# coop-columb/two-tower-amazon-recommender

Hardware: AMD Instinct MI355X
Metric: user-item pairs/sec (train step) + embedding-gather HBM GB/s, 1/2/4/8 MI355X (higher is better)
Workload: dtype f32; 1 GPU; cfg3: 5000000 users x 10000000 items, emb_dim 128, towers 128->256->128, batch 8192, in-batch sampled softmax T=0.1, sgd lr 1e-3, ids U; global_batch=8192, parallelism=single GPU

## Files before the change

two_tower_amazon_recommender_amd/csrc/score.hip:

```cpp
#include "common.h"

namespace {

using tt::f32x4;
using tt::f32x16;
typedef __bf16 bf16x4 __attribute__((ext_vector_type(4)));
typedef __bf16 bf16x8 __attribute__((ext_vector_type(8)));
typedef short s16x4 __attribute__((ext_vector_type(4)));

constexpr float kLog2e = 1.44269504088896340736f;
constexpr float kLn2 = 0.69314718055994530942f;
constexpr float kNegBig = -1.0e30f;

enum { MODE_FWD = 0, MODE_BWD = 1, MODE_FUSED = 2, MODE_RANK = 3, MODE_FUSED_S = 4, MODE_BWD_S = 5,
       MODE_FUSED_S_NC = 6, MODE_BWD_S_NR = 7 };
constexpr int base_mode(int m) { return m == MODE_FUSED_S_NC ? (int)MODE_FUSED_S : (m == MODE_BWD_S_NR ? (int)MODE_BWD_S : m); }
template <bool B> struct BoolC { static constexpr bool value = B; };
constexpr float kRescaleThr = 8.0f;

struct ScoreArgs {
  const float* R;
  const float* K;
  int64_t n_r, n_c;
  int64_t diag;
  float c1;
  const float* a_r;
  const float* s_r;
  const float* a_c;
  const float* s_c;
  const int64_t* id_r;
  const int64_t* id_c;
  int nsplit;
  int64_t c_per_split;
  float* part_m;
  float* part_l;
  float* pos2;
  float* slab;
  const float* h_r;
  const float* h_c;
  const int64_t* pos_idx;
  int32_t* part_cnt;
  float* S;
  int64_t ldS;
};

template <int D, int PREC>
struct Geo {
  static constexpr int LS = D + 4;
  static constexpr int NG = D / 8;
  static constexpr int NB = D / 32;
  static constexpr int KS = D / 16;
  static constexpr int HALF_B = 32 * 256;
  static constexpr int PIECE_B = (D / 128) * HALF_B;
  static constexpr int TILE_F = PREC == 0 ? 32 * LS : 3 * PIECE_B / 4;
  static constexpr int BUF_F = TILE_F + 160;
  static constexpr int LDS_BYTES = 2 * BUF_F * 4;
};

struct Bf3 {
  __bf16 hi, mid, lo;
};
__device__ __forceinline__ Bf3 split3(float x) {
  Bf3 o;
  o.hi = (__bf16)x;
  const float r1 = x - (float)o.hi;
  o.mid = (__bf16)r1;
  o.lo = (__bf16)(r1 - (float)o.mid);
  return o;
}

__device__ __forceinline__ int img_off(int row, int ch) { return 256 * row + 16 * (ch ^ (((row & 3) << 2) | ((row >> 2) & 3))); }

constexpr int kBwdSWaves = 2;
constexpr int kSPrefetch = 2;
#ifndef TT_LOOP_LAMBDA
#define TT_LOOP_LAMBDA 0
#endif
constexpr int kTilesPerBarrier = 2;
constexpr int kTilesPerBarrierBwdS = kTilesPerBarrier;
template <int D, int MODE, int PREC>
constexpr int tiles_per_barrier() {
  if (PREC == 0 && D <= 128 && MODE == MODE_BWD_S) return kTilesPerBarrierBwdS;
  return (PREC == 0 && D <= 128 && (MODE == MODE_BWD || MODE == MODE_FUSED || MODE == MODE_FUSED_S))
             ? kTilesPerBarrier : 1;
}

template <int D, int MODE, int PREC>
constexpr bool split_d() {
  return PREC == 1 && D == 256 && (MODE == MODE_BWD || MODE == MODE_FUSED || MODE == MODE_FUSED_S);
}
template <int D, int MODE, bool HAS_IDS, bool HAS_HN, int PREC>
constexpr int rf_lds_groups() {
  if (PREC == 0 && D == 256 && (MODE == MODE_FUSED || MODE == MODE_FUSED_S) && (HAS_IDS || HAS_HN))
    return (HAS_IDS && HAS_HN) ? 10 : (HAS_HN ? 8 : 5);
  if (PREC == 0 && D == 128 && MODE == MODE_BWD && HAS_IDS && HAS_HN) return 2;
  return 0;
}
template <int D, int MODE, int PREC, int WAVES>
constexpr int rows_per_wg() { return (split_d<D, MODE, PREC>() ? WAVES / 2 : WAVES) * 32; }

template <int D, int MODE_T, bool HAS_IDS, bool HAS_HN, int WAVES, int PREC>
__global__ __launch_bounds__(WAVES * 64, (WAVES == 8 ? 2 : (D <= 128 ? ((base_mode(MODE_T) == MODE_BWD_S && PREC == 0) ? kBwdSWaves : 2) : 1))) void score_kernel(ScoreArgs p) {
  constexpr int MODE = base_mode(MODE_T);
  constexpr bool FAST = MODE_T != MODE;
  static_assert(!FAST || (PREC == 0 && !HAS_IDS && !HAS_HN), "the fast forms: exact f32, no ids, no hard negatives");
  constexpr BoolC<false> GEN{};
  constexpr BoolC<true> FULL_TILE{};
  constexpr bool NO_AC = FAST && MODE == MODE_FUSED_S;
  constexpr bool NO_ROW = FAST && MODE == MODE_BWD_S;
  constexpr bool IS_FUSED = MODE == MODE_FUSED || MODE == MODE_FUSED_S;
  constexpr bool IS_BWD = MODE == MODE_BWD || MODE == MODE_BWD_S;
  constexpr bool FROM_S = MODE == MODE_BWD_S, TO_S = MODE == MODE_FUSED_S;
  using G_ = Geo<D, PREC>;
  constexpr int LS = G_::LS, NG = G_::NG, NB = G_::NB, TILE_F = G_::TILE_F, BUF_F = G_::BUF_F;
  constexpr int HALF_B = G_::HALF_B, PIECE_B = G_::PIECE_B;
  constexpr bool SPLIT = split_d<D, MODE, PREC>();
  constexpr int KS = SPLIT ? G_::KS / 2 : G_::KS;
  constexpr int NBW = SPLIT ? NB / 2 : NB;
  static_assert(PREC == 0 || D % 128 == 0, "bf16x3: dim 128 / 256 only (whole [32][128] bf16 images)");
  constexpr int ROW4 = D / 4;
  constexpr int THREADS = WAVES * 64;
  constexpr int NV = (32 * ROW4 + THREADS - 1) / THREADS;
  extern __shared__ __attribute__((aligned(16))) float smem[];

  const int tid = threadIdx.x;
  const int lane = tid & 63;
  const int wave = FAST ? __builtin_amdgcn_readfirstlane(tid >> 6) : tid >> 6;
  const int h = lane >> 5;
  const int ln = lane & 31;

  const int split = __builtin_amdgcn_readfirstlane((int)(blockIdx.x % (unsigned)p.nsplit));
  const int64_t rblk = __builtin_amdgcn_readfirstlane((int)(blockIdx.x / (unsigned)p.nsplit));
  const int hw = SPLIT ? (wave & 1) : 0;
  const int64_t r0w = rblk * rows_per_wg<D, MODE, PREC, WAVES>() + (SPLIT ? wave >> 1 : wave) * 32;
  const int64_t r = r0w + ln;
  const bool r_ok = r < p.n_r;
  const int64_t c_begin = (int64_t)split * p.c_per_split;
  int64_t c_end = c_begin + p.c_per_split;
  if (c_end > p.n_c) c_end = p.n_c;
  const int ntiles = __builtin_amdgcn_readfirstlane(c_end > c_begin ? (int)((c_end - c_begin + 31) >> 5) : 0);
  const int nfull = __builtin_amdgcn_readfirstlane(c_end > c_begin ? (int)((c_end - c_begin) >> 5) : 0);

// ... 40 lines not shown
  }
  const float ar = (!NO_ROW && (IS_BWD || MODE == MODE_RANK) && p.a_r != nullptr && r_ok) ? p.a_r[r] : 0.f;
  const float sr = (!NO_ROW && IS_BWD && p.s_r != nullptr && r_ok) ? p.s_r[r] : 1.f;
  int64_t idr = 0;
  if constexpr (HAS_IDS) idr = r_ok ? p.id_r[r] : (int64_t)-1;
  const int64_t cpos = p.pos_idx != nullptr ? (r_ok ? p.pos_idx[r] : (int64_t)-1) : r + p.diag;

  f32x4 st[NV];
  float st_a = 0.f, st_s = 0.f, st_h = -3.0e38f;
  constexpr bool hn = HAS_HN;
  const float hr = (HAS_HN && p.h_r != nullptr && r_ok) ? p.h_r[r] : -3.0e38f;
  int64_t st_id = -2;
  constexpr int RPJ = THREADS / ROW4 > 0 ? THREADS / ROW4 : 1;
  const int st_row = tid / ROW4, st_col4 = tid % ROW4;
  const f32x4* kp = reinterpret_cast<const f32x4*>(p.K) + c_begin * ROW4;
  const bool has_ac = p.a_c != nullptr, has_sc = p.s_c != nullptr, has_hc = HAS_HN && p.h_c != nullptr;
  const float* acp = (has_ac ? p.a_c : p.K) + c_begin;
  const float* scp = (has_sc ? p.s_c : p.K) + c_begin;
  const float* hcp = (has_hc ? p.h_c : p.K) + c_begin;
  const int64_t* idp = nullptr;
  if constexpr (HAS_IDS) idp = p.id_c + c_begin;
  const int ncols = (int)(c_end - c_begin);

  constexpr bool ST_FULL = NV * THREADS == 32 * ROW4;
  auto load_tile = [&](int t, auto full) {
    constexpr bool FULL = decltype(full)::value;
    const f32x4* src = kp + (int64_t)t * (32 * ROW4);
    if constexpr (FULL) {
      static_assert(ST_FULL || NV == 1, "threads past row 31 exist only where a thread stages one float4");
      const unsigned off0 = (unsigned)((ST_FULL ? st_row : (st_row < 31 ? st_row : 31)) * ROW4 + st_col4);
#pragma unroll
      for (int j = 0; j < NV; ++j) st[j] = (src + (ST_FULL ? j * RPJ * ROW4 : 0))[off0];
      const unsigned c31 = (unsigned)(tid < 31 ? tid : 31);
      if constexpr (!NO_AC) st_a = (acp + 32 * (int64_t)t)[c31];
      if constexpr (IS_BWD) st_s = (scp + 32 * (int64_t)t)[c31];
      return;
    }
    const int nvalid = ncols - 32 * t;
    const int last = (nvalid < 32 ? nvalid : 32) - 1;
#pragma unroll
    for (int j = 0; j < NV; ++j) {
      const int row = st_row + j * RPJ;
      st[j] = src[(row < last ? row : last) * ROW4 + st_col4];
    }
    const int c = 32 * t + (tid < last ? tid : last);
    if constexpr (!NO_AC) st_a = acp[c];
    if constexpr (HAS_HN) st_h = hcp[c];
    if constexpr (IS_BWD) st_s = scp[c];
    if constexpr (HAS_IDS) st_id = idp[c];
  };
  auto store_tile = [&](int t, int buf, auto full) {
    constexpr bool FULL = decltype(full)::value;
    float* T = smem + buf * BUF_F;
    const int nvalid = ncols - 32 * t;
    if constexpr (!FULL) {
#pragma unroll
      for (int j = 0; j < NV; ++j) st[j] = (st_row + j * RPJ < nvalid) ? st[j] : f32x4{0.f, 0.f, 0.f, 0.f};
    }
    if constexpr (!ST_FULL) {
#pragma unroll
      for (int j = 0; j < NV; ++j) asm volatile("" : : "v"(st[j]));
    }
    if constexpr (PREC == 0) {
      float* dst = T + st_row * LS + st_col4 * 4;
#pragma unroll
      for (int j = 0; j < NV; ++j)
        if (ST_FULL || st_row + j * RPJ < 32) *reinterpret_cast<f32x4*>(dst + j * RPJ * LS) = st[j];
    } else {
      char* img = reinterpret_cast<char*>(T);
      const int d0 = 4 * st_col4;
      const int sub = (d0 >> 7) * HALF_B + 8 * ((d0 >> 2) & 1), ch = (d0 & 127) >> 3;
#pragma unroll
      for (int j = 0; j < NV; ++j) {
        const int row = st_row + j * RPJ;
        if (ST_FULL || row < 32) {
          bf16x4 q0, q1, q2;
#pragma unroll
          for (int e = 0; e < 4; ++e) {
            const Bf3 u = split3(st[j][e]);
            q0[e] = u.hi; q1[e] = u.mid; q2[e] = u.lo;
          }
          char* dst = img + sub + img_off(row, ch);
          *reinterpret_cast<bf16x4*>(dst) = q0;
          *reinterpret_cast<bf16x4*>(dst + PIECE_B) = q1;
          *reinterpret_cast<bf16x4*>(dst + 2 * PIECE_B) = q2;
        }
      }
    }
    if constexpr (NO_AC) {
      return;
    } else if constexpr (NO_ROW) {
      asm volatile("" : : "v"(st_a));
      asm volatile("" : : "v"(st_s));
      if (tid < 32) {
        const bool ok = FULL || tid < nvalid;
        T[TILE_F + tid] = ok ? st_a : kNegBig;
        T[TILE_F + 32 + tid] = ok ? st_s : 0.f;
      }
      return;
    }
    asm volatile("" : : "v"(st_a));
    if constexpr (IS_BWD) asm volatile("" : : "v"(st_s));
    if constexpr (HAS_HN) asm volatile("" : : "v"(st_h));
    if constexpr (HAS_IDS) asm volatile("" : : "v"(st_id));
    if (tid < 32) {
      const bool ok = tid < nvalid;
      T[TILE_F + tid] = ok ? (has_ac ? st_a : 0.f) : kNegBig;
      T[TILE_F + 32 + tid] = ok ? ((IS_BWD && has_sc) ? st_s : 1.f) : 0.f;
      if constexpr (HAS_HN) T[TILE_F + 128 + tid] = (ok && has_hc) ? st_h : -3.0e38f;
      if constexpr (HAS_IDS) reinterpret_cast<int64_t*>(T + TILE_F + 64)[tid] = ok ? st_id : (int64_t)-2;
    }
  };

  const bool frag_ok = __builtin_amdgcn_readfirstlane((int)(r0w < p.n_r)) != 0;
  auto store_S = [&](int t, const f32x16& X) {
    if (!frag_ok) return;
    const int64_t ctile = (c_begin >> 5) + t;
    if constexpr (FAST) {
      float* blk_u = p.S + (ctile * p.ldS + (r0w >> 5)) * 1024;
      const unsigned lo = (unsigned)(ln * 32 + 4 * h);
#pragma unroll
      for (int g = 0; g < 4; ++g) *reinterpret_cast<f32x4*>(blk_u + (lo + 8u * g)) = f32x4{X[4 * g], X[4 * g + 1], X[4 * g + 2], X[4 * g + 3]};
// ... 10 lines not shown
    f32x4* mine = reinterpret_cast<f32x4*>(xch + wave * 1024) + lane;
    const f32x4* other = reinterpret_cast<const f32x4*>(xch + (wave ^ 1) * 1024) + lane;
#pragma unroll
    for (int g = 0; g < 4; ++g) mine[64 * g] = f32x4{X[4 * g], X[4 * g + 1], X[4 * g + 2], X[4 * g + 3]};
    __syncthreads();
#pragma unroll
    for (int g = 0; g < 4; ++g) {
      const f32x4 o = other[64 * g];
#pragma unroll
      for (int i = 0; i < 4; ++i) X[4 * g + i] += o[i];
    }
  };
  auto load_S = [&](int t, f32x16& X) {
    const int64_t q0 = c_begin + 32 * (int64_t)t;
    if constexpr (FAST) {
      const float* blk_u = p.S + ((frag_ok ? (r0w >> 5) : 0) * p.ldS + (q0 >> 5)) * 1024;
      const unsigned lo = (unsigned)(4 * h * 32 + ln);
#pragma unroll
      for (int reg = 0; reg < 16; ++reg) X[reg] = blk_u[lo + (unsigned)(tt::acc_row(reg, 0) * 32)];
      return;
    }
    const float* blk = p.S + ((frag_ok ? (r0w >> 5) : 0) * p.ldS + (q0 >> 5)) * 1024 + 4 * h * 32 + ln;
#pragma unroll
    for (int reg = 0; reg < 16; ++reg) X[reg] = blk[tt::acc_row(reg, 0) * 32];
  };
  auto mask_S = [&](int t, const f32x16& Xin) -> f32x16 {
    const int nq_left = ncols - 32 * t;
    f32x16 X;
#pragma unroll
    for (int reg = 0; reg < 16; ++reg) X[reg] = (r_ok && (tt::acc_row(reg, 0) + 4 * h) < nq_left) ? Xin[reg] : 0.f;
    return X;
  };
  auto clamp_tile = [&](int t) { return t < ntiles ? t : ntiles - 1; };

  float run_m = kNegBig, run_l = 0.f, pos = 0.f;
  int cnt = 0;
  bool have_pos = false;
  f32x16 G[NBW];
  if constexpr (IS_BWD || IS_FUSED) {
#pragma unroll
    for (int b = 0; b < NBW; ++b)
#pragma unroll
      for (int i = 0; i < 16; ++i) G[b][i] = 0.f;
  }

#pragma unroll
  for (int t0 = 0; t0 < TPB; ++t0)
    if (t0 < ntiles) {
      load_tile(t0, GEN);
      store_tile(t0, t0, GEN);
    }
  __syncthreads();
  auto gemm1 = [&](const float* T) -> f32x16 {
    f32x16 X;
#pragma unroll
    for (int i = 0; i < 16; ++i) X[i] = 0.f;
    if constexpr (PREC == 1) {
      const char* img = reinterpret_cast<const char*>(T);
      auto frag = [&](int ks, bf16x8& f_hi, bf16x8& f_mid, bf16x8& f_lo, bf16x8& r_lo) {
        const int off = (SPLIT ? hw : (ks >> 3)) * HALF_B + img_off(ln, 2 * (ks & 7) + h);
        f_hi = *reinterpret_cast<const bf16x8*>(img + off);
        f_mid = *reinterpret_cast<const bf16x8*>(img + PIECE_B + off);
        f_lo = *reinterpret_cast<const bf16x8*>(img + 2 * PIECE_B + off);
        if constexpr (RLO_LDS) r_lo = rlo[ks * 64];
      };
      bf16x8 a_hi, a_mid, a_lo, b_lo = {};
// ... 6 lines not shown
        X = __builtin_amdgcn_mfma_f32_32x32x16_bf16(a_lo, rp[0][ks], X, 0, 0, 0);
        X = __builtin_amdgcn_mfma_f32_32x32x16_bf16(a_hi, b_lo, X, 0, 0, 0);
        X = __builtin_amdgcn_mfma_f32_32x32x16_bf16(a_mid, rp[1][ks], X, 0, 0, 0);
        X = __builtin_amdgcn_mfma_f32_32x32x16_bf16(a_mid, rp[0][ks], X, 0, 0, 0);
        X = __builtin_amdgcn_mfma_f32_32x32x16_bf16(a_hi, rp[1][ks], X, 0, 0, 0);
        X = __builtin_amdgcn_mfma_f32_32x32x16_bf16(a_hi, rp[0][ks], X, 0, 0, 0);
        a_hi = n_hi; a_mid = n_mid; a_lo = n_lo; b_lo = nb_lo;
        __builtin_amdgcn_sched_barrier(0);
      }
    } else {
      const float* arow = T + ln * LS + 4 * h;
      f32x4 a_cur = *reinterpret_cast<const f32x4*>(arow);
#pragma unroll
      for (int g = 0; g < NG; ++g) {
        f32x4 a_nxt = a_cur;
        if (g + 1 < NG) a_nxt = *reinterpret_cast<const f32x4*>(arow + 8 * (g + 1));
        f32x4 rg;
        if constexpr (RFL > 0) { if (g >= RFR) rg = rfl[(g - RFR) * 64]; else rg = rf[g < RFR ? g : 0]; } else rg = rf[g];
        X = __builtin_amdgcn_mfma_f32_32x32x2f32(a_cur[0], rg[0], X, 0, 0, 0);
        X = __builtin_amdgcn_mfma_f32_32x32x2f32(a_cur[1], rg[1], X, 0, 0, 0);
        X = __builtin_amdgcn_mfma_f32_32x32x2f32(a_cur[2], rg[2], X, 0, 0, 0);
        X = __builtin_amdgcn_mfma_f32_32x32x2f32(a_cur[3], rg[3], X, 0, 0, 0);
        a_cur = a_nxt;
        __builtin_amdgcn_sched_barrier(0);
      }
    }
    return X;
  };

  auto epilogue = [&](const float* T, int t, const f32x16& X, float (&coef)[16], auto full) {
    constexpr bool FULL = decltype(full)::value;
    const int64_t c0 = c_begin + 32 * (int64_t)t;
    float ac[16], sc[16];
#pragma unroll
    for (int q = 0; q < 4; ++q) {
      if constexpr (NO_AC) {
      } else {
        const f32x4 va = *reinterpret_cast<const f32x4*>(T + TILE_F + 8 * q + 4 * h);
#pragma unroll
        for (int i = 0; i < 4; ++i) ac[4 * q + i] = va[i];
      }
      if constexpr (IS_BWD) {
        const f32x4 vs = *reinterpret_cast<const f32x4*>(T + TILE_F + 32 + 8 * q + 4 * h);
#pragma unroll
        for (int i = 0; i < 4; ++i) sc[4 * q + i] = vs[i];
      }
    }
    float hth[16];
    if constexpr (hn) {
#pragma unroll
      for (int q = 0; q < 4; ++q) {
        const f32x4 vh = *reinterpret_cast<const f32x4*>(T + TILE_F + 128 + 8 * q + 4 * h);
#pragma unroll
        for (int i = 0; i < 4; ++i) hth[4 * q + i] = fmaxf(vh[i], hr);
      }
    }
    bool diag_tile;
    if (p.pos_idx != nullptr) {
      const int64_t dd0 = cpos - c0;
      diag_tile = __any(dd0 >= 0 && dd0 < 32) != 0;
    } else {
      diag_tile = (c0 < r0w + p.diag + 32) && (c0 + 32 > r0w + p.diag);
    }
    int dloc = -100;
    if (diag_tile) {
      const int64_t dd = cpos - c0;
      dloc = (dd >= 0 && dd < 32) ? (int)dd - 4 * h : -100;
    }
    auto take_pos = [&](bool hit, float v) {
      if constexpr (HAS_IDS) {
        if (hit) { pos = v; have_pos = true; }
      } else {
        pos = hit ? v : pos;
        have_pos = have_pos || hit;
      }
// ... 153 lines not shown
      auto read_k = [&](int reg, f32x4& k0, f32x4& k1) {
        const float* krow = kbase + tt::acc_row(reg, 0) * LS;
        if constexpr (NB == 8) {
          k0 = *reinterpret_cast<const f32x4*>(krow);
          k1 = *reinterpret_cast<const f32x4*>(krow + 4);
        } else if constexpr (NB == 4) {
          k0 = *reinterpret_cast<const f32x4*>(krow);
        } else if constexpr (NB == 2) {
          const float2 k2 = *reinterpret_cast<const float2*>(krow);
          k0[0] = k2.x; k0[1] = k2.y;
        } else {
          k0[0] = krow[0];
        }
      };
      read_k(0, kc0, kc1);
#pragma unroll
      for (int reg = 0; reg < 16; ++reg) {
        f32x4 kn0 = kc0, kn1 = kc1;
        if (reg + 1 < 16) read_k(reg + 1, kn0, kn1);
#pragma unroll
        for (int b = 0; b < (NB < 4 ? NB : 4); ++b)
          G[b] = __builtin_amdgcn_mfma_f32_32x32x2f32(kc0[b], coef[reg], G[b], 0, 0, 0);
        if constexpr (NB == 8) {
#pragma unroll
          for (int b = 0; b < 4; ++b)
            G[4 + b] = __builtin_amdgcn_mfma_f32_32x32x2f32(kc1[b], coef[reg], G[4 + b], 0, 0, 0);
        }
        kc0 = kn0; kc1 = kn1;
        __builtin_amdgcn_sched_barrier(0);
      }
    }
  };

  if constexpr (FROM_S && kSPrefetch == 2) {
    f32x16 xa, xb;
#pragma unroll
    for (int i = 0; i < 16; ++i) { xa[i] = 0.f; xb[i] = 0.f; }
    auto tile_step = [&](int t, f32x16& xs_t) {
      if constexpr (PREC == 1) load_tile(clamp_tile(t + 1), GEN);
      const float* T = smem + (t % NBUF) * BUF_F;
      const f32x16 X = mask_S(t, xs_t);
      float coef[16];
      epilogue(T, t, X, coef, GEN);
      if constexpr (PREC == 0) load_tile(clamp_tile(t + TPB), GEN);
      load_S(clamp_tile(t + 2), xs_t);
      gemm2(T, coef);
      store_tile(t + TPB, (t + TPB) % NBUF, GEN);
      if ((t % TPB) == TPB - 1) __syncthreads();
    };
    auto full_step = [&](int t, f32x16& xs_t) {
      const float* T = smem + (t % NBUF) * BUF_F;
      float coef[16];
      epilogue(T, t, xs_t, coef, FULL_TILE);
      load_tile(t + TPB, FULL_TILE);
      load_S(t + 2, xs_t);
      gemm2(T, coef);
      store_tile(t + TPB, (t + TPB) % NBUF, FULL_TILE);
      if ((t % TPB) == TPB - 1) __syncthreads();
    };
    if (ntiles > 0) {
      load_S(0, xa);
      load_S(clamp_tile(1), xb);
      int t = 0;
      if constexpr (FAST) {
        static_assert(TPB <= 2, "full_step prefetches at most two tiles ahead");
        const int nfast = (nfull > 2 ? nfull - 2 : 0) & ~1;
        for (; t < nfast; t += 2) {
          full_step(t, xa);
          full_step(t + 1, xb);
        }
      }
      for (; t + 1 < ntiles; t += 2) {
        tile_step(t, xa);
        tile_step(t + 1, xb);
      }
      if (t < ntiles) tile_step(t, xa);
    }
  } else {
    f32x16 xs;
#pragma unroll
    for (int i = 0; i < 16; ++i) xs[i] = 0.f;
    if constexpr (FROM_S) { if (ntiles > 0) load_S(0, xs); }
    int t_first = 0;
    if constexpr (FAST) {
      static_assert(!FROM_S && !SPLIT, "the fast form of pass 1");
      const int nfast = nfull > TPB ? nfull - TPB : 0;
      for (int t = 0; t < nfast; ++t) {
        const float* T = smem + (t % NBUF) * BUF_F;
        const f32x16 X = gemm1(T);
        store_S(t, X);
        float coef[16];
        epilogue(T, t, X, coef, FULL_TILE);
        load_tile(t + TPB, FULL_TILE);
        gemm2(T, coef);
        store_tile(t + TPB, (t + TPB) % NBUF, FULL_TILE);
        if ((t % TPB) == TPB - 1) __syncthreads();
      }
      t_first = nfast;
    }
#if TT_LOOP_LAMBDA
    auto tile_step = [&](int t) {
      if constexpr (MODE == MODE_FWD || MODE == MODE_RANK || PREC == 1) load_tile(clamp_tile(t + 1), GEN);
      const float* T = smem + (t % NBUF) * BUF_F;
      f32x16 X;
      if constexpr (FROM_S) X = mask_S(t, xs); else X = gemm1(T);
      if constexpr (SPLIT) exchange(X);
      if constexpr (TO_S) store_S(t, X);
      float coef[16];
      epilogue(T, t, X, coef, GEN);
// ... 26 lines not shown
      }
      store_tile(t + TPB, (t + TPB) % NBUF, GEN);
      if ((t % TPB) == TPB - 1) __syncthreads();
    }
#endif
  }

  if constexpr (IS_FUSED) {
    const float L = run_l + __shfl_xor(run_l, 32);
    if (r_ok && hw == 0) {
      if (h == 0) {
        p.part_m[(int64_t)split * p.n_r + r] = run_m;
        p.part_l[(int64_t)split * p.n_r + r] = L;
      }
      if (have_pos) p.pos2[r] = pos;
    }
  }
  if constexpr (MODE == MODE_RANK) {
    const int total = cnt + __shfl_xor(cnt, 32);
    if (r_ok && h == 0) p.part_cnt[(int64_t)split * p.n_r + r] = total;
  } else if constexpr (MODE == MODE_FWD) {
    const float om = __shfl_xor(run_m, 32);
    const float ol = __shfl_xor(run_l, 32);
    const float M = fmaxf(run_m, om);
    const float L = run_l * __builtin_amdgcn_exp2f(run_m - M) + ol * __builtin_amdgcn_exp2f(om - M);
    if (r_ok) {
      if (h == 0) {
        p.part_m[(int64_t)split * p.n_r + r] = M;
        p.part_l[(int64_t)split * p.n_r + r] = L;
      }
      if (have_pos) p.pos2[r] = pos;
    }
  } else {
    if (r_ok) {
      float* out = p.slab + ((int64_t)split * p.n_r + r) * D + 128 * hw;
      if constexpr (PREC == 1) {
#pragma unroll
        for (int b = 0; b < NBW; ++b)
#pragma unroll
          for (int g = 0; g < 4; ++g)
            *reinterpret_cast<f32x4*>(out + 32 * b + 8 * g + 4 * h) = f32x4{G[b][4 * g], G[b][4 * g + 1], G[b][4 * g + 2], G[b][4 * g + 3]};
      } else
#pragma unroll
      for (int reg = 0; reg < 16; ++reg) {
        const int i = tt::acc_row(reg, 0) + 4 * h;
        if constexpr (NB == 8) {
          *reinterpret_cast<f32x4*>(out + 8 * i) = f32x4{G[0][reg], G[1][reg], G[2][reg], G[3][reg]};
          *reinterpret_cast<f32x4*>(out + 8 * i + 4) = f32x4{G[4][reg], G[5][reg], G[6][reg], G[7][reg]};
        } else if constexpr (NB == 4) {
          *reinterpret_cast<f32x4*>(out + 4 * i) = f32x4{G[0][reg], G[1][reg], G[2][reg], G[3][reg]};
        } else if constexpr (NB == 2) {
          *reinterpret_cast<float2*>(out + 2 * i) = float2{G[0][reg], G[1][reg]};
        } else {
          out[i] = G[0][reg];
        }
      }
    }
  }
}


__global__ __launch_bounds__(256) void prob_bias_kernel(const float* __restrict__ prob, float* __restrict__ out, int64_t n) {
  const int64_t i = (int64_t)blockIdx.x * 256 + threadIdx.x;
  if (i < n) out[i] = -__log2f(fminf(fmaxf(prob[i], 1e-6f), 1.0f));
}

__global__ __launch_bounds__(256) void bwd_prep_kernel(const float* __restrict__ lse, const float* __restrict__ w,
                                                       float* __restrict__ a, float* __restrict__ s, int64_t n,
// ... 225 lines not shown
    for (int64_t r0 = t; r0 < n_rows; r0 += 8 * 1024) {
      float v[8][4];
#pragma unroll
      for (int i = 0; i < 8; ++i)
#pragma unroll
        for (int j = 0; j < 4; ++j) {
          const int64_t r = r0 + 1024 * i + 256 * j;
          v[i][j] = r < n_rows ? per_row[r] : 0.f;
        }
#pragma unroll
      for (int i = 0; i < 8; ++i)
#pragma unroll
        for (int j = 0; j < 4; ++j)
          if (r0 + 1024 * i + 256 * j < n_rows) a[j] += v[i][j];
    }
    red[t] = (a[0] + a[2]) + (a[1] + a[3]);
    __syncthreads();
    for (int s2 = 128; s2 > 0; s2 >>= 1) {
      if (t < s2) red[t] += red[t + s2];
      __syncthreads();
    }
    if (t == 0) loss[0] = red[0];
    return;
  }
  const int64_t nblk = per_row != nullptr ? gridDim.x - 1 : gridDim.x;
  const int64_t stride = nblk * 256;
  for (int64_t i = (int64_t)blockIdx.x * 256 + threadIdx.x; i < n4; i += stride) {
    f32x4 a = slab[i];
    for (int s = 1; s < nsplit; ++s) a += slab[(int64_t)s * n4 + i];
    out[i] = a;
  }
}


constexpr int kScoreWaves = 4;
constexpr int kScoreWgs = 512;
constexpr int kBwdSWgs = 512;
int choose_nsplit_pow2(int64_t n_r, int64_t n_c, int target_wgs = kScoreWgs) {
  const int64_t nrb = (n_r + 32 * kScoreWaves - 1) / (32 * kScoreWaves);
  int ns = 1;
  while (nrb * ns < target_wgs && (int64_t)ns * 2 * 64 <= n_c && ns < 64) ns *= 2;
  return ns;
}

int choose_nsplit(int64_t n_r, int64_t n_c, int rows_per_wg = 32 * kScoreWaves, int slots = kScoreWgs) {
  const int64_t nrb = (n_r + rows_per_wg - 1) / rows_per_wg;
  int best = 1;
  double best_cost = 0.0;
  for (int ns = 1; ns <= 64; ++ns) {
    if (ns > 1 && (int64_t)ns * 64 > n_c) break;
    const int64_t rounds = (nrb * ns + slots - 1) / slots;
    const double cost = (double)rounds / ns * (1.0 + 0.005 * ns);
    if (ns == 1 || cost < best_cost - 1e-12) { best = ns; best_cost = cost; }
  }
  return best;
}

int64_t align_up(int64_t x, int64_t a) { return (x + a - 1) / a * a; }

struct WsLayout {
  int ns_q, ns_c;
  int ns_cs;
  int64_t off_bias, off_aq, off_sq, off_hq, off_pm, off_pl, off_pos, off_slab, off_S, total_no_S, total;
};

WsLayout ws_layout(int64_t nq, int64_t nc, int32_t dim) {
// ... 4 lines not shown
    w.ns_cs = choose_nsplit(nc, nq, 256, 256);
  } else {
    w.ns_q = choose_nsplit_pow2(nq, nc);
    w.ns_c = choose_nsplit_pow2(nc, nq);
    w.ns_cs = choose_nsplit_pow2(nc, nq, kBwdSWgs);
  }
  int64_t o = 0;
  w.off_bias = o; o = align_up(o + nc * 4, 256);
  w.off_aq = o;   o = align_up(o + nq * 4, 256);
  w.off_sq = o;   o = align_up(o + nq * 4, 256);
  w.off_hq = o;   o = align_up(o + nq * 4, 256);
  w.off_pm = o;   o = align_up(o + (int64_t)w.ns_q * nq * 4, 256);
  w.off_pl = o;   o = align_up(o + (int64_t)w.ns_q * nq * 4, 256);
  w.off_pos = o;  o = align_up(o + nq * 4, 256);
  w.off_slab = o;
  const int64_t slab_q = (int64_t)w.ns_q * nq * dim * 4, slab_c = (int64_t)(w.ns_c > w.ns_cs ? w.ns_c : w.ns_cs) * nc * dim * 4;
  o = align_up(o + (slab_q > slab_c ? slab_q : slab_c), 256);
  w.total_no_S = o;
  w.off_S = o;
  o = align_up(o + ((nq + 31) / 32) * ((nc + 31) / 32) * 4096, 256);
  w.total = o;
  return w;
}

constexpr int kBwdSWgWaves = 8;
constexpr int kFusedSWgWaves = 4;
template <int D, int MODE_T, int PREC = 0>
constexpr int waves_for() {
  constexpr int MODE = base_mode(MODE_T);
  return (PREC == 1 && D == 128) ? 8 : (PREC == 1 ? 4 : ((MODE == MODE_BWD_S && D <= 128) ? kBwdSWgWaves
                                                         : ((MODE == MODE_FUSED_S && D <= 128) ? kFusedSWgWaves : kScoreWaves)));
}

template <int D, int MODE, int PREC = 0>
int launch_score(const ScoreArgs& a_in, hipStream_t stream) {
  constexpr int W = waves_for<D, MODE, PREC>();
  constexpr int RPW = rows_per_wg<D, MODE, PREC, W>();
  const int64_t nrb = (a_in.n_r + RPW - 1) / RPW;
  const int64_t blocks = nrb * a_in.nsplit;
  const int lds_base = Geo<D, PREC>::LDS_BYTES * tiles_per_barrier<D, MODE, PREC>() +
                  ((PREC == 1 && W == 8) ? W * Geo<D, PREC>::KS * 64 * 16 : 0) +
                  (split_d<D, MODE, PREC>() ? W * 4096 : 0);
  const bool has_ids = a_in.id_c != nullptr;
  const bool has_hn = (a_in.h_r != nullptr) || (a_in.h_c != nullptr);
  const ScoreArgs& a = a_in;
  auto go = [&](auto kern, int rfl_groups = 0) -> int {
    const int lds = lds_base + W * rfl_groups * 64 * 16;
    if (lds > 64 * 1024) {
      if (hipFuncSetAttribute(reinterpret_cast<const void*>(kern), hipFuncAttributeMaxDynamicSharedMemorySize, lds) != hipSuccess)
        return tt::fail(TT_ERR_LAUNCH, "hipFuncSetAttribute(LDS %d) failed", lds);
    }
    constexpr const char* tag = MODE == MODE_FWD ? "score_fwd" : ((MODE == MODE_BWD || MODE == MODE_BWD_S) ? "score_bwd"
                                : ((MODE == MODE_FUSED || MODE == MODE_FUSED_S) ? "score_fused" : "score_rank"));
    tt::launch(tag, kern, dim3((unsigned)blocks), dim3(W * 64), (unsigned)lds, stream, a);
    return tt::check_launch(tag);
  };
  if constexpr (PREC == 0 && (MODE == MODE_FUSED_S || MODE == MODE_BWD_S)) {
    if (!has_ids && !has_hn && a.pos_idx == nullptr) {
      if constexpr (MODE == MODE_FUSED_S) {
        if constexpr (D == 64 || D == 128) {
          if (a.a_c == nullptr) return go(score_kernel<D, MODE_FUSED_S_NC, false, false, W, 0>);
        }
      } else {
        if (a.a_r == nullptr && a.s_r == nullptr && a.a_c != nullptr && a.s_c != nullptr)
          return go(score_kernel<D, MODE_BWD_S_NR, false, false, W, 0>);
      }
    }
  }
  if (has_ids && has_hn) return go(score_kernel<D, MODE, true, true, W, PREC>, rf_lds_groups<D, MODE, true, true, PREC>());
  if (has_ids) return go(score_kernel<D, MODE, true, false, W, PREC>, rf_lds_groups<D, MODE, true, false, PREC>());
  if (has_hn) return go(score_kernel<D, MODE, false, true, W, PREC>, rf_lds_groups<D, MODE, false, true, PREC>());
  return go(score_kernel<D, MODE, false, false, W, PREC>);
}

template <int MODE>
int dispatch_score(int prec, int32_t dim, const ScoreArgs& a, hipStream_t stream) {
  if (prec == 1) {
    if constexpr (MODE == MODE_BWD) return tt::fail(TT_ERR_UNSUPPORTED, "retrieval (bf16x3): no separate backward pass");
    else switch (dim) {
      case 128: return launch_score<128, MODE, 1>(a, stream);
      case 256: return launch_score<256, MODE, 1>(a, stream);
      default: return tt::fail(TT_ERR_UNSUPPORTED, "retrieval (bf16x3): dim %d not in {128,256}", dim);
    }
  }
  switch (dim) {
    case 32: return launch_score<32, MODE>(a, stream);
    case 64: return launch_score<64, MODE>(a, stream);
    case 128: return launch_score<128, MODE>(a, stream);
    case 256: return launch_score<256, MODE>(a, stream);
    default: return tt::fail(TT_ERR_UNSUPPORTED, "retrieval: dim %d not in {32,64,128,256}", dim);
  }
}

enum WsNeed { WS_RANK, WS_NO_S, WS_FULL };

int check_common(const char* fn, const float* q, const float* c, int64_t nq, int64_t nc, int32_t dim,
// ... 26 lines not shown
  const int64_t* ids_q = cand_ids != nullptr ? cand_ids + diag_offset : nullptr;
  ScoreArgs a{};
  if (side == STATIONARY_Q) {
    a.R = q; a.K = c; a.n_r = nq; a.n_c = nc; a.diag = diag_offset;
    a.id_r = ids_q; a.id_c = cand_ids;
  } else {
    a.R = c; a.K = q; a.n_r = nc; a.n_c = nq; a.diag = -diag_offset;
    a.id_r = cand_ids; a.id_c = ids_q;
  }
  a.c1 = kLog2e * inv_temperature;
  a.nsplit = nsplit;
  a.c_per_split = align_up((a.n_c + nsplit - 1) / nsplit, 32);
  return a;
}

ScoreArgs dc_pass_args(const float* q, const float* c, int64_t nq, int64_t nc, int64_t diag_offset, float inv_temperature,
                       int nsplit, const int64_t* cand_ids, const float* bias, const float* aq, const float* sq,
                       const float* hq, float* slab, float* smat) {
  ScoreArgs a = pass_args(STATIONARY_C, q, c, nq, nc, diag_offset, inv_temperature, nsplit, cand_ids);
  a.a_r = bias; a.s_r = nullptr; a.a_c = aq; a.s_c = sq;
  a.h_c = hq;
  a.slab = slab;
  if (smat != nullptr) { a.S = smat; a.ldS = (nq + 31) / 32; }
  return a;
}

int reduce_slabs(const char* what, const float* slab, float* out, int64_t n, int32_t dim, int nsplit, const float* per_row,
                 int64_t n_rows, float* loss, hipStream_t stream) {
  const int64_t n4 = n * dim / 4;
  const int64_t blocks = (n4 + 255) / 256 < 2048 ? (n4 + 255) / 256 : 2048;
  tt::launch("score_aux", reduce_slabs_kernel, dim3((unsigned)blocks + (per_row != nullptr ? 1 : 0)), dim3(256), 0, stream,
             reinterpret_cast<const f32x4*>(slab), reinterpret_cast<f32x4*>(out), n4, nsplit, per_row, n_rows, loss);
  return tt::check_launch(what);
}

}

extern "C" int32_t tt_retrieval_num_splits(int64_t nq, int64_t nc, int32_t dim, int32_t pass) {
  if (nq <= 0 || nc <= 0 || dim <= 0 || pass < 0 || pass > 2) return 0;
  const WsLayout w = ws_layout(nq, nc, dim);
  return pass == 0 ? w.ns_q : (pass == 1 ? w.ns_c : w.ns_cs);
}

extern "C" int64_t tt_retrieval_workspace_bytes(int64_t nq, int64_t nc, int32_t dim) {
  if (nq <= 0 || nc <= 0 || dim <= 0) return 0;
  return ws_layout(nq, nc, dim).total;
}

extern "C" int64_t tt_retrieval_fwd_workspace_bytes(int64_t nq, int64_t nc, int32_t dim) {
  if (nq <= 0 || nc <= 0 || dim <= 0) return 0;
  return ws_layout(nq, nc, dim).total_no_S;
}

extern "C" int64_t tt_retrieval_rank_workspace_bytes(int64_t nq, int64_t nc, int32_t dim) {
  if (nq <= 0 || nc <= 0 || dim <= 0) return 0;
  return ws_layout(nq, nc, dim).off_pl;
}

static int retrieval_fwd(const char* fn, int prec, const float* q, const float* c, int64_t nq, int64_t nc, int32_t dim,
                         int64_t diag_offset, float inv_temperature, const float* sample_weight,
                         const float* cand_prob, const int64_t* cand_ids, const float* hard_thr,
                         void* workspace, int64_t workspace_bytes, float* lse, float* per_row, float* loss,
                         tt_stream_t stream_) {
  int rc = check_common(fn, q, c, nq, nc, dim, diag_offset, workspace, workspace_bytes, WS_NO_S);
  if (rc != TT_OK) return rc;
  TT_REQUIRE(lse && per_row && loss, "%s: null output pointer", fn);
// ... 74 lines not shown
  const ScoreArgs a = dc_pass_args(q, c, nq, nc, diag_offset, inv_temperature, w.ns_c, cand_ids, bias, aq, sq, hq, slab, nullptr);
  if ((rc = dispatch_score<MODE_BWD>(0, dim, a, stream)) != TT_OK) return rc;
  return reduce_slabs("reduce_slabs(dc)", slab, dc, nc, dim, a.nsplit, nullptr, 0, nullptr, stream);
}

static int retrieval_fwd_bwd(const char* fn, int prec, const float* q, const float* c, int64_t nq, int64_t nc, int32_t dim,
                             int64_t diag_offset, float inv_temperature, const float* sample_weight,
                             const float* cand_prob, const int64_t* cand_ids, const float* hard_thr,
                             float grad_scale, void* workspace, int64_t workspace_bytes, float* lse,
                             float* per_row, float* loss, float* dq, float* dc, tt_stream_t stream_) {
  int rc = check_common(fn, q, c, nq, nc, dim, diag_offset, workspace, workspace_bytes, WS_FULL);
  if (rc != TT_OK) return rc;
  TT_REQUIRE(lse && per_row && loss && dq && dc, "%s: null output pointer", fn);
  TT_REQUIRE(tt::aligned16(dq) && tt::aligned16(dc), "%s: dq/dc must be 16-byte aligned", fn);
  hipStream_t stream = tt::as_stream(stream_);
  const WsLayout w = ws_layout(nq, nc, dim);
  char* ws = static_cast<char*>(workspace);
  float* aq = reinterpret_cast<float*>(ws + w.off_aq);
  float* sq = reinterpret_cast<float*>(ws + w.off_sq);
  float* slab = reinterpret_cast<float*>(ws + w.off_slab);
  float* smat = reinterpret_cast<float*>(ws + w.off_S);
  const float* bias;
  if ((rc = column_bias(cand_prob, nc, workspace, w, stream, &bias)) != TT_OK) return rc;
  {
    ScoreArgs a = pass_args(STATIONARY_Q, q, c, nq, nc, diag_offset, inv_temperature, w.ns_q, cand_ids);
    a.a_c = bias;
    a.h_r = hard_thr;
    a.S = smat; a.ldS = (nq + 31) / 32;
    a.part_m = reinterpret_cast<float*>(ws + w.off_pm);
    a.part_l = reinterpret_cast<float*>(ws + w.off_pl);
    a.pos2 = reinterpret_cast<float*>(ws + w.off_pos);
    a.slab = slab;
    if ((rc = dispatch_score<MODE_FUSED_S>(prec, dim, a, stream)) != TT_OK) return rc;
    int lpr_log2 = 3;
    while ((1 << lpr_log2) < dim / 4) ++lpr_log2;
    const int rpb = 256 >> lpr_log2;
    tt::launch("score_aux", fused_combine_kernel, dim3((unsigned)((nq + rpb - 1) / rpb)), dim3(256), 0, stream, a.part_m, a.part_l, a.pos2,
                       sample_weight, reinterpret_cast<const f32x4*>(slab),
                       reinterpret_cast<const f32x4*>(c + diag_offset * dim), nq, dim / 4, lpr_log2, a.nsplit,
                       inv_temperature * grad_scale, lse, per_row, aq, sq, reinterpret_cast<f32x4*>(dq));
    if ((rc = tt::check_launch("fused_combine")) != TT_OK) return rc;
  }
  float* hq = nullptr;
  if (hard_thr != nullptr) {
    hq = reinterpret_cast<float*>(ws + w.off_hq);
    hipLaunchKernelGGL(hn_shift_kernel, dim3((unsigned)((nq + 255) / 256)), dim3(256), 0, stream, hard_thr, aq, hq, nq);
    if ((rc = tt::check_launch("hn_shift")) != TT_OK) return rc;
  }
  const ScoreArgs a = dc_pass_args(q, c, nq, nc, diag_offset, inv_temperature, w.ns_cs, cand_ids, bias, aq, sq, hq, slab, smat);
  if ((rc = dispatch_score<MODE_BWD_S>(prec, dim, a, stream)) != TT_OK) return rc;
  return reduce_slabs("reduce_slabs(dc)", slab, dc, nc, dim, a.nsplit, per_row, nq, loss, stream);
}

extern "C" int tt_retrieval_fwd_bwd_f32(const float* q, const float* c, int64_t nq, int64_t nc, int32_t dim,
                                        int64_t diag_offset, float inv_temperature, const float* sample_weight,
                                        const float* cand_prob, const int64_t* cand_ids, const float* hard_thr,
                                        float grad_scale, void* workspace, int64_t workspace_bytes, float* lse,
                                        float* per_row, float* loss, float* dq, float* dc, tt_stream_t stream) {
  return retrieval_fwd_bwd("tt_retrieval_fwd_bwd_f32", 0, q, c, nq, nc, dim, diag_offset, inv_temperature, sample_weight, cand_prob,
                           cand_ids, hard_thr, grad_scale, workspace, workspace_bytes, lse, per_row, loss, dq, dc, stream);
}

extern "C" int tt_retrieval_fwd_bwd_bf16x3_f32(const float* q, const float* c, int64_t nq, int64_t nc, int32_t dim,
                                               int64_t diag_offset, float inv_temperature, const float* sample_weight,
                                               const float* cand_prob, const int64_t* cand_ids, const float* hard_thr,
                                               float grad_scale, void* workspace, int64_t workspace_bytes, float* lse,
// ... 75 lines not shown
```

Baseline: 15.51 million pairs/s.

## Fuse query-side softmax combine into dc backward pass and reduce dc from S blocks

Adds a MODE_BWD_S_CMB score-kernel variant. Each workgroup recomputes per-row logsumexp statistics from the forward split partials into LDS tables, then interleaves the dq combine (weighted sum of slab partials plus the positive term) with the dc GEMM tile loop. This removes the separate fused_combine launch and its aq/sq round-trip. The dc partials are written into the now-free S buffer in block layout and summed by a new reduce_dc_blocks kernel. In exchange the stats work is repeated in every row block, LDS use grows, and the path only applies to exact f32 with dim 64/128 and no ids, sampling correction or hard negatives.

```diff
diff --git a/two_tower_amazon_recommender_amd/csrc/score.hip b/two_tower_amazon_recommender_amd/csrc/score.hip
--- a/two_tower_amazon_recommender_amd/csrc/score.hip
+++ b/two_tower_amazon_recommender_amd/csrc/score.hip
@@ -13,8 +13,11 @@
 constexpr float kNegBig = -1.0e30f;
 
 enum { MODE_FWD = 0, MODE_BWD = 1, MODE_FUSED = 2, MODE_RANK = 3, MODE_FUSED_S = 4, MODE_BWD_S = 5,
-       MODE_FUSED_S_NC = 6, MODE_BWD_S_NR = 7 };
-constexpr int base_mode(int m) { return m == MODE_FUSED_S_NC ? (int)MODE_FUSED_S : (m == MODE_BWD_S_NR ? (int)MODE_BWD_S : m); }
+       MODE_FUSED_S_NC = 6, MODE_BWD_S_NR = 7,
+       MODE_BWD_S_CMB = 8 };
+constexpr int base_mode(int m) {
+  return m == MODE_FUSED_S_NC ? (int)MODE_FUSED_S : ((m == MODE_BWD_S_NR || m == MODE_BWD_S_CMB) ? (int)MODE_BWD_S : m);
+}
 template <bool B> struct BoolC { static constexpr bool value = B; };
 constexpr float kRescaleThr = 8.0f;
 
@@ -42,6 +45,15 @@
   int32_t* part_cnt;
   float* S;
   int64_t ldS;
+  const float* cmb_w;
+  const float* cmb_cpos;
+  const float* cmb_slab;
+  float* cmb_lse;
+  float* cmb_per_row;
+  float* cmb_dq;
+  int cmb_ns;
+  int cmb_rows;
+  float cmb_scale;
 };
 
 template <int D, int PREC>
@@ -108,6 +120,7 @@
   constexpr BoolC<true> FULL_TILE{};
   constexpr bool NO_AC = FAST && MODE == MODE_FUSED_S;
   constexpr bool NO_ROW = FAST && MODE == MODE_BWD_S;
+  constexpr bool CMB = MODE_T == MODE_BWD_S_CMB;
   constexpr bool IS_FUSED = MODE == MODE_FUSED || MODE == MODE_FUSED_S;
   constexpr bool IS_BWD = MODE == MODE_BWD || MODE == MODE_BWD_S;
   constexpr bool FROM_S = MODE == MODE_BWD_S, TO_S = MODE == MODE_FUSED_S;
@@ -214,8 +227,8 @@
 #pragma unroll
       for (int j = 0; j < NV; ++j) st[j] = (src + (ST_FULL ? j * RPJ * ROW4 : 0))[off0];
       const unsigned c31 = (unsigned)(tid < 31 ? tid : 31);
-      if constexpr (!NO_AC) st_a = (acp + 32 * (int64_t)t)[c31];
-      if constexpr (IS_BWD) st_s = (scp + 32 * (int64_t)t)[c31];
+      if constexpr (!NO_AC && !CMB) st_a = (acp + 32 * (int64_t)t)[c31];
+      if constexpr (IS_BWD && !CMB) st_s = (scp + 32 * (int64_t)t)[c31];
       return;
     }
     const int nvalid = ncols - 32 * t;
@@ -226,9 +239,9 @@
       st[j] = src[(row < last ? row : last) * ROW4 + st_col4];
     }
     const int c = 32 * t + (tid < last ? tid : last);
-    if constexpr (!NO_AC) st_a = acp[c];
+    if constexpr (!NO_AC && !CMB) st_a = acp[c];
     if constexpr (HAS_HN) st_h = hcp[c];
-    if constexpr (IS_BWD) st_s = scp[c];
+    if constexpr (IS_BWD && !CMB) st_s = scp[c];
     if constexpr (HAS_IDS) st_id = idp[c];
   };
   auto store_tile = [&](int t, int buf, auto full) {
@@ -269,7 +282,7 @@
         }
       }
     }
-    if constexpr (NO_AC) {
+    if constexpr (NO_AC || CMB) {
       return;
     } else if constexpr (NO_ROW) {
       asm volatile("" : : "v"(st_a));
@@ -346,6 +359,10 @@
     return X;
   };
   auto clamp_tile = [&](int t) { return t < ntiles ? t : ntiles - 1; };
+  float* tab_a = smem + NBUF * BUF_F;
+  float* tab_s = tab_a + (CMB ? (int)p.c_per_split : 0);
+  float* cmb_inv = tab_s + (CMB ? (int)p.c_per_split : 0);
+  float* cmb_e = cmb_inv + (CMB ? p.cmb_rows : 0);
 
   float run_m = kNegBig, run_l = 0.f, pos = 0.f;
   int cnt = 0;
@@ -418,15 +435,22 @@
     constexpr bool FULL = decltype(full)::value;
     const int64_t c0 = c_begin + 32 * (int64_t)t;
     float ac[16], sc[16];
+    int tab_o = 32 * t + 4 * h;
+    if constexpr (CMB) asm volatile("" : "+v"(tab_o));
 #pragma unroll
     for (int q = 0; q < 4; ++q) {
       if constexpr (NO_AC) {
+      } else if constexpr (CMB) {
+        const f32x4 va = *reinterpret_cast<const f32x4*>(tab_a + tab_o + 8 * q);
+        const f32x4 vs = *reinterpret_cast<const f32x4*>(tab_s + tab_o + 8 * q);
+#pragma unroll
+        for (int i = 0; i < 4; ++i) { ac[4 * q + i] = va[i]; sc[4 * q + i] = vs[i]; }
       } else {
         const f32x4 va = *reinterpret_cast<const f32x4*>(T + TILE_F + 8 * q + 4 * h);
 #pragma unroll
         for (int i = 0; i < 4; ++i) ac[4 * q + i] = va[i];
       }
-      if constexpr (IS_BWD) {
+      if constexpr (IS_BWD && !CMB) {
         const f32x4 vs = *reinterpret_cast<const f32x4*>(T + TILE_F + 32 + 8 * q + 4 * h);
 #pragma unroll
         for (int i = 0; i < 4; ++i) sc[4 * q + i] = vs[i];
@@ -646,49 +670,215 @@
     }
   };
 
+  const int cmb_lo = CMB ? (int)rblk * p.cmb_rows : 0;
+  auto cmb_stats = [&]() {
+    constexpr int U = 8, RR = 2;
+    const int ns = p.cmb_ns, last = ns - 1;
+    const unsigned nq = (unsigned)p.n_c;
+    auto at = [](const float* base, unsigned byte_off) { return *reinterpret_cast<const float*>(reinterpret_cast<const char*>(base) + byte_off); };
+    for (int i0 = tid; i0 < (int)p.c_per_split; i0 += RR * THREADS) {
+      bool ok[RR];
+      unsigned rowb[RR];
+      float pm0[RR][U], pl0[RR][U], wr[RR], p2[RR];
+#pragma unroll
+      for (int rr = 0; rr < RR; ++rr) {
+        const int i = i0 + rr * THREADS;
+        ok[rr] = i < (int)p.c_per_split && c_begin + i < c_end;
+        rowb[rr] = (ok[rr] ? (unsigned)c_begin + (unsigned)i : nq - 1u) * 4u;
+      }
+#pragma unroll
+      for (int u = 0; u < U; ++u) {
+        const unsigned sb = (unsigned)(u < last ? u : last) * nq;
+#pragma unroll
+        for (int rr = 0; rr < RR; ++rr) {
+          pm0[rr][u] = at(p.part_m + sb, rowb[rr]);
+          pl0[rr][u] = at(p.part_l + sb, rowb[rr]);
+        }
+      }
+#pragma unroll
+      for (int rr = 0; rr < RR; ++rr) {
+        wr[rr] = (p.cmb_w != nullptr ? at(p.cmb_w, rowb[rr]) : 1.0f);
+        p2[rr] = at(p.pos2, rowb[rr]);
+      }
+#pragma unroll
+      for (int rr = 0; rr < RR; ++rr) {
+        const int i = i0 + rr * THREADS;
+        const int il = i - cmb_lo;
+        const bool mine = il >= 0 && il < p.cmb_rows && i < (int)p.c_per_split;
+        float M = kNegBig;
+#pragma unroll
+        for (int u = 0; u < U; ++u) M = fmaxf(M, pm0[rr][u]);
+        for (int s0 = U; s0 < ns; s0 += U) {
+          float pm[U];
+#pragma unroll
+          for (int u = 0; u < U; ++u) pm[u] = at(p.part_m + (unsigned)(s0 + u < last ? s0 + u : last) * nq, rowb[rr]);
+#pragma unroll
+          for (int u = 0; u < U; ++u) M = fmaxf(M, pm[u]);
+        }
+        float L = 0.f;
+        float e0[U];
+#pragma unroll
+        for (int u = 0; u < U; ++u) {
+          e0[u] = __builtin_amdgcn_exp2f(pm0[rr][u] - M);
+          if (u < ns) L += pl0[rr][u] * e0[u];
+        }
+        if (mine) {
+#pragma unroll
+          for (int u = 0; u < U; ++u)
+            if (u < ns) cmb_e[il * ns + u] = e0[u];
+        }
+        for (int s0 = U; s0 < ns; s0 += U) {
+          float pm[U], pl[U];
+#pragma unroll
+          for (int u = 0; u < U; ++u) {
+            const unsigned sb = (unsigned)(s0 + u < last ? s0 + u : last) * nq;
+            pm[u] = at(p.part_m + sb, rowb[rr]);
+            pl[u] = at(p.part_l + sb, rowb[rr]);
+          }
+#pragma unroll
+          for (int u = 0; u < U; ++u)
+            if (s0 + u < ns) {
+              const float e = __builtin_amdgcn_exp2f(pm[u] - M);
+              L += pl[u] * e;
+              if (mine) cmb_e[il * ns + s0 + u] = e;
+            }
+        }
+        const float lse2 = M + __log2f(L);
+        if (i < (int)p.c_per_split) {
+          tab_a[i] = ok[rr] ? -lse2 : kNegBig;
+          tab_s[i] = ok[rr] ? wr[rr] * p.cmb_scale : 0.f;
+        }
+        if (mine) cmb_inv[il] = 1.0f / L;
+        if (rblk == 0 && ok[rr]) {
+          *reinterpret_cast<float*>(reinterpret_cast<char*>(p.cmb_lse) + rowb[rr]) = lse2 * kLn2;
+          *reinterpret_cast<float*>(reinterpret_cast<char*>(p.cmb_per_row) + rowb[rr]) = (lse2 - p2[rr]) * kLn2 * wr[rr];
+        }
+      }
+    }
+  };
+  const int cmb_ko = CMB ? (p.cmb_rows * ROW4 + THREADS - 1) / THREADS : 0;
+  const int cmb_items = cmb_ko * (p.cmb_ns + 1);
+  struct CmbSlot { f32x4 v; float ef; int sf; };
+  CmbSlot cmb_a{f32x4{0.f, 0.f, 0.f, 0.f}, 0.f, 0}, cmb_b{f32x4{0.f, 0.f, 0.f, 0.f}, 0.f, 0};
+  int cmb_j = 0, cmb_si = 0;
+  int cmb_oi = tid, cmb_oc = tid;
+  unsigned cmb_offi = 0;
+  int cmb_eoi = 0;
+  const f32x4* cmb_base = reinterpret_cast<const f32x4*>(p.cmb_slab);
+  f32x4 cmb_acc = f32x4{0.f, 0.f, 0.f, 0.f};
+  auto cmb_out = [&](int o, int& rl, bool& ok) -> unsigned {
+    const int r_loc = o / ROW4;
+    const int rows_left = (int)(c_end - c_begin) - cmb_lo;
+    ok = r_loc < p.cmb_rows && r_loc < rows_left;
+    rl = ok ? r_loc : 0;
+    const int row_s = ok ? cmb_lo + r_loc : 0;
+    return (unsigned)((int)c_begin + row_s) * (unsigned)ROW4 + (unsigned)(o % ROW4);
+  };
+  auto cmb_init = [&]() {
+    int rl; bool ok;
+    cmb_offi = cmb_out(cmb_oi, rl, ok) * 16u;
+    cmb_eoi = rl * p.cmb_ns;
+  };
+  auto cmb_load = [&](CmbSlot& sl) {
+    const f32x4* base = cmb_si < p.cmb_ns ? cmb_base : reinterpret_cast<const f32x4*>(p.cmb_cpos);
+    sl.v = *reinterpret_cast<const f32x4*>(reinterpret_cast<const char*>(base) + cmb_offi);
+  };
+  auto cmb_advance = [&](CmbSlot& sl) {
+    sl.ef = cmb_e[cmb_eoi + cmb_si];
+    sl.sf = cmb_si;
+    ++cmb_si;
+    cmb_base += p.n_c * ROW4;
+    ++cmb_j;
+    if (cmb_si > p.cmb_ns) {
+      cmb_si = 0;
+      cmb_base = reinterpret_cast<const f32x4*>(p.cmb_slab);
+      cmb_oi += THREADS;
+      int rl; bool ok;
+      cmb_offi = cmb_out(cmb_oi, rl, ok) * 16u;
+      cmb_eoi = rl * p.cmb_ns;
+    }
+  };
+  auto cmb_consume = [&](const CmbSlot& sl) {
+    f32x4 acc = cmb_acc + sl.v * sl.ef;
+    if (sl.sf == p.cmb_ns) {
+      int rl; bool ok;
+      const unsigned off = cmb_out(cmb_oc, rl, ok);
+      const float inv_l = cmb_inv[rl], sr = tab_s[ok ? cmb_lo + rl : 0];
+      if (ok) reinterpret_cast<f32x4*>(p.cmb_dq)[off] = (cmb_acc * inv_l - sl.v) * sr;
+      acc = f32x4{0.f, 0.f, 0.f, 0.f};
+      cmb_oc += THREADS;
+    }
+    cmb_acc = acc;
+  };
+  auto cmb_step = [&](CmbSlot& sl) {
+    cmb_consume(sl);
+    cmb_load(sl);
+    cmb_advance(sl);
+  };
+
   if constexpr (FROM_S && kSPrefetch == 2) {
     f32x16 xa, xb;
 #pragma unroll
     for (int i = 0; i < 16; ++i) { xa[i] = 0.f; xb[i] = 0.f; }
-    auto tile_step = [&](int t, f32x16& xs_t) {
+    auto tile_step = [&](int t, f32x16& xs_t, CmbSlot& sl) {
       if constexpr (PREC == 1) load_tile(clamp_tile(t + 1), GEN);
       const float* T = smem + (t % NBUF) * BUF_F;
       const f32x16 X = mask_S(t, xs_t);
       float coef[16];
       epilogue(T, t, X, coef, GEN);
       if constexpr (PREC == 0) load_tile(clamp_tile(t + TPB), GEN);
+      if constexpr (CMB) cmb_step(sl);
       load_S(clamp_tile(t + 2), xs_t);
       gemm2(T, coef);
       store_tile(t + TPB, (t + TPB) % NBUF, GEN);
       if ((t % TPB) == TPB - 1) __syncthreads();
     };
-    auto full_step = [&](int t, f32x16& xs_t) {
+    auto full_step = [&](int t, f32x16& xs_t, CmbSlot& sl) {
       const float* T = smem + (t % NBUF) * BUF_F;
       float coef[16];
       epilogue(T, t, xs_t, coef, FULL_TILE);
       load_tile(t + TPB, FULL_TILE);
+      if constexpr (CMB) cmb_step(sl);
       load_S(t + 2, xs_t);
       gemm2(T, coef);
       store_tile(t + TPB, (t + TPB) % NBUF, FULL_TILE);
       if ((t % TPB) == TPB - 1) __syncthreads();
     };
     if (ntiles > 0) {
+      if constexpr (CMB) {
+        cmb_init();
+        cmb_load(cmb_a);
+      }
       load_S(0, xa);
       load_S(clamp_tile(1), xb);
+      if constexpr (CMB) {
+        cmb_stats();
+        __syncthreads();
+        cmb_advance(cmb_a);
+        cmb_load(cmb_b);
+        cmb_advance(cmb_b);
+      }
       int t = 0;
       if constexpr (FAST) {
         static_assert(TPB <= 2, "full_step prefetches at most two tiles ahead");
         const int nfast = (nfull > 2 ? nfull - 2 : 0) & ~1;
         for (; t < nfast; t += 2) {
-          full_step(t, xa);
-          full_step(t + 1, xb);
+          full_step(t, xa, cmb_a);
+          full_step(t + 1, xb, cmb_b);
         }
       }
       for (; t + 1 < ntiles; t += 2) {
-        tile_step(t, xa);
-        tile_step(t + 1, xb);
-      }
-      if (t < ntiles) tile_step(t, xa);
+        tile_step(t, xa, cmb_a);
+        tile_step(t + 1, xb, cmb_b);
+      }
+      if (t < ntiles) tile_step(t, xa, cmb_a);
+      if constexpr (CMB) {
+        bool odd = (ntiles & 1) != 0;
+        while (cmb_j < cmb_items + 2) {
+          if (odd) cmb_step(cmb_b); else cmb_step(cmb_a);
+          odd = !odd;
+        }
+      }
     }
   } else {
     f32x16 xs;
@@ -781,8 +971,9 @@
       if (have_pos) p.pos2[r] = pos;
     }
   } else {
-    if (r_ok) {
+    if (r_ok && !(CMB && ntiles == 0)) {
       float* out = p.slab + ((int64_t)split * p.n_r + r) * D + 128 * hw;
+      if constexpr (CMB) out = p.S + ((r0w >> 5) * p.ldS + (c_begin >> 5)) * 1024 + ln * D;
       if constexpr (PREC == 1) {
 #pragma unroll
         for (int b = 0; b < NBW; ++b)
@@ -1074,6 +1265,50 @@
   }
 }
 
+__global__ __launch_bounds__(256) void reduce_dc_blocks_kernel(const f32x4* __restrict__ S, f32x4* __restrict__ out, int64_t n4,
+                                                               int d4_log2, int64_t ldS, int64_t tiles_per_split, int n_live,
+                                                               int nsplit, const float* __restrict__ per_row, int64_t n_rows,
+                                                               float* __restrict__ loss) {
+  if (blockIdx.x == gridDim.x - 1) {
+    __shared__ float red[256];
+    const int t = threadIdx.x;
+    float a[4] = {0.f, 0.f, 0.f, 0.f};
+    for (int64_t r0 = t; r0 < n_rows; r0 += 8 * 1024) {
+      float v[8][4];
+#pragma unroll
+      for (int i = 0; i < 8; ++i)
+#pragma unroll
+        for (int j = 0; j < 4; ++j) {
+          const int64_t r = r0 + 1024 * i + 256 * j;
+          v[i][j] = r < n_rows ? per_row[r] : 0.f;
+        }
+#pragma unroll
+      for (int i = 0; i < 8; ++i)
+#pragma unroll
+        for (int j = 0; j < 4; ++j)
+          if (r0 + 1024 * i + 256 * j < n_rows) a[j] += v[i][j];
+    }
+    red[t] = (a[0] + a[2]) + (a[1] + a[3]);
+    __syncthreads();
+    for (int s2 = 128; s2 > 0; s2 >>= 1) {
+      if (t < s2) red[t] += red[t + s2];
+      __syncthreads();
+    }
+    if (t == 0) loss[0] = red[0];
+    return;
+  }
+  const int64_t stride = (int64_t)(gridDim.x - 1) * 256;
+  const f32x4 zero = f32x4{0.f, 0.f, 0.f, 0.f};
+  for (int64_t i = (int64_t)blockIdx.x * 256 + threadIdx.x; i < n4; i += stride) {
+    const int64_t r = i >> d4_log2;
+    const f32x4* src = S + ((r >> 5) * ldS) * 256 + (((r & 31) << d4_log2) + (i & ((1 << d4_log2) - 1)));
+    f32x4 a = src[0];
+    for (int s = 1; s < n_live; ++s) a += src[(int64_t)s * tiles_per_split * 256];
+    for (int s = n_live; s < nsplit; ++s) a += zero;
+    out[i] = a;
+  }
+}
+
 
 constexpr int kScoreWaves = 4;
 constexpr int kScoreWgs = 512;
@@ -1144,6 +1379,8 @@
                                                          : ((MODE == MODE_FUSED_S && D <= 128) ? kFusedSWgWaves : kScoreWaves)));
 }
 
+int64_t cmb_lds_bytes(const ScoreArgs& a) { return (2 * a.c_per_split + (int64_t)a.cmb_rows * (1 + a.cmb_ns) + 4) * 4; }
+
 template <int D, int MODE, int PREC = 0>
 int launch_score(const ScoreArgs& a_in, hipStream_t stream) {
   constexpr int W = waves_for<D, MODE, PREC>();
@@ -1156,8 +1393,8 @@
   const bool has_ids = a_in.id_c != nullptr;
   const bool has_hn = (a_in.h_r != nullptr) || (a_in.h_c != nullptr);
   const ScoreArgs& a = a_in;
-  auto go = [&](auto kern, int rfl_groups = 0) -> int {
-    const int lds = lds_base + W * rfl_groups * 64 * 16;
+  auto go = [&](auto kern, int rfl_groups = 0, int extra_lds = 0) -> int {
+    const int lds = lds_base + W * rfl_groups * 64 * 16 + extra_lds;
     if (lds > 64 * 1024) {
       if (hipFuncSetAttribute(reinterpret_cast<const void*>(kern), hipFuncAttributeMaxDynamicSharedMemorySize, lds) != hipSuccess)
         return tt::fail(TT_ERR_LAUNCH, "hipFuncSetAttribute(LDS %d) failed", lds);
@@ -1174,6 +1411,10 @@
           if (a.a_c == nullptr) return go(score_kernel<D, MODE_FUSED_S_NC, false, false, W, 0>);
         }
       } else {
+        if constexpr (D == 64 || D == 128) {
+          if (a.cmb_dq != nullptr) return go(score_kernel<D, MODE_BWD_S_CMB, false, false, W, 0>, 0, (int)cmb_lds_bytes(a));
+        }
+        if (a.cmb_dq != nullptr) return tt::fail(TT_ERR_UNSUPPORTED, "retrieval: no combining dc pass at dim %d", D);
         if (a.a_r == nullptr && a.s_r == nullptr && a.a_c != nullptr && a.s_c != nullptr)
           return go(score_kernel<D, MODE_BWD_S_NR, false, false, W, 0>);
       }
@@ -1266,6 +1507,24 @@
   tt::launch("score_aux", reduce_slabs_kernel, dim3((unsigned)blocks + (per_row != nullptr ? 1 : 0)), dim3(256), 0, stream,
              reinterpret_cast<const f32x4*>(slab), reinterpret_cast<f32x4*>(out), n4, nsplit, per_row, n_rows, loss);
   return tt::check_launch(what);
+}
+
+bool cmb_applies(int prec, int32_t dim, const float* cand_prob, const int64_t* cand_ids, const float* hard_thr, int ns_q,
+                 ScoreArgs& a, int* n_live) {
+  if (prec != 0 || cand_prob != nullptr || cand_ids != nullptr || hard_thr != nullptr) return false;
+  if (dim != 64 && dim != 128) return false;
+  const int64_t nq = a.n_c, cps = a.c_per_split, need = dim / 32;
+  const int64_t live = (nq + cps - 1) / cps;
+  const int64_t last_tiles = (nq - (live - 1) * cps + 31) / 32;
+  if (cps / 32 < need || last_tiles < need) return false;
+  if (nq * dim * 4 >= ((int64_t)1 << 32) || (int64_t)ns_q * nq >= ((int64_t)1 << 29)) return false;
+  const int64_t nrb = (a.n_r + 32 * kBwdSWgWaves - 1) / (32 * kBwdSWgWaves);
+  a.cmb_rows = (int)((cps + nrb - 1) / nrb);
+  a.cmb_ns = ns_q;
+  const int64_t lds = (int64_t)Geo<128, 0>::LDS_BYTES * kTilesPerBarrierBwdS + cmb_lds_bytes(a);
+  if (lds > 160 * 1024) { a.cmb_rows = 0; a.cmb_ns = 0; return false; }
+  *n_live = (int)live;
+  return true;
 }
 
 }
@@ -1406,6 +1665,25 @@
     a.pos2 = reinterpret_cast<float*>(ws + w.off_pos);
     a.slab = slab;
     if ((rc = dispatch_score<MODE_FUSED_S>(prec, dim, a, stream)) != TT_OK) return rc;
+    ScoreArgs b = dc_pass_args(q, c, nq, nc, diag_offset, inv_temperature, w.ns_cs, nullptr, nullptr, aq, sq, nullptr, slab, smat);
+    int n_live = 0;
+    if (cmb_applies(prec, dim, cand_prob, cand_ids, hard_thr, a.nsplit, b, &n_live)) {
+      b.part_m = a.part_m; b.part_l = a.part_l; b.pos2 = a.pos2;
+      b.cmb_w = sample_weight;
+      b.cmb_cpos = c + diag_offset * dim;
+      b.cmb_slab = slab;
+      b.cmb_lse = lse; b.cmb_per_row = per_row; b.cmb_dq = dq;
+      b.cmb_scale = inv_temperature * grad_scale;
+      if ((rc = dispatch_score<MODE_BWD_S>(prec, dim, b, stream)) != TT_OK) return rc;
+      int d4_log2 = 0;
+      while ((1 << d4_log2) < dim / 4) ++d4_log2;
+      const int64_t n4 = nc * (dim / 4);
+      const int64_t blocks = (n4 + 255) / 256 < 2048 ? (n4 + 255) / 256 : 2048;
+      tt::launch("score_aux", reduce_dc_blocks_kernel, dim3((unsigned)blocks + 1), dim3(256), 0, stream,
+                 reinterpret_cast<const f32x4*>(smat), reinterpret_cast<f32x4*>(dc), n4, d4_log2, b.ldS, b.c_per_split / 32, n_live,
+                 b.nsplit, per_row, nq, loss);
+      return tt::check_launch("reduce_dc_blocks");
+    }
     int lpr_log2 = 3;
     while ((1 << lpr_log2) < dim / 4) ++lpr_log2;
     const int rpb = 256 >> lpr_log2;
```

After: 15.58 million pairs/s, median of 6. About the same (+0.4%).
